# tennisonliu/bayesian-neural-network

Hardware: AMD Instinct MI355X
Metric: MC-forward-samples/sec + KL-elements/sec, 784-1200-1200-10 BNN (higher is better)
Workload: dtype bf16

## Files before the change

### bayesian-neural-network_amd/csrc/bbb_linear.hip

```cpp
#include "bnn_device.h"
#include "bnn_fin.h"
#include "bbb_sample_body.h"
#include "bbb_block_gemm.h"
#include "../../include/bnn_hip.h"
#include <string.h>

namespace bnn {

struct BbbK {
  const void* x;
  long x_sstride;
  const float* w_mu;
  const float* w_rho;
  const float* w_sigma;
  const float* b_mu;
  const float* b_rho;
  const float* eps_w;
  const float* eps_b;
  float* eps_w_dump;
  float* eps_b_dump;
  void* y;
  float4* ws;
  int S, B, K, N;
  __bf16* y16;
// ... 581 lines not shown
      if (threadIdx.x == 0) fp->ks_stats[(size_t)s * KS + ks] = make_float4(own0, own1, own2, 0.f);
      asm volatile("s_waitcnt vmcnt(0)" ::: "memory");
      __syncthreads();
      uint32_t* flag = reinterpret_cast<uint32_t*>(part);
      if (threadIdx.x == 0) {
        __builtin_amdgcn_fence(__ATOMIC_RELEASE, "agent");
        asm volatile("s_waitcnt vmcnt(0)" ::: "memory");
        const uint32_t tk = __hip_atomic_fetch_add(fp->ks_ticket + s, 1u, __ATOMIC_RELAXED, __HIP_MEMORY_SCOPE_AGENT);
        const uint32_t last = (tk == (uint32_t)KS - 1u) ? 1u : 0u;
        if (last) {
          __builtin_amdgcn_fence(__ATOMIC_ACQUIRE, "agent");
          asm volatile("s_waitcnt vmcnt(0)" ::: "memory");
        }
        *flag = last;
      }
      __syncthreads();
      BNN_STAMP(7);
      if (*flag == 0u) return true;
      __syncthreads();
      const float* tiles = fp->ks_tiles + (size_t)s * KS * (128 * 16);
      float4 q4 = make_float4(0.f, 0.f, 0.f, 0.f);
      if ((int)threadIdx.x < KS) q4 = fp->ks_stats[(size_t)s * KS + threadIdx.x];
      for (int it = threadIdx.x; it < 128 * 4; it += blockDim.x) {
        const int brow = it >> 2, fg = it & 3;
        f32x4 v = f32x4{0.f, 0.f, 0.f, 0.f};
        for (int j = 0; j < KS; ++j) v += *reinterpret_cast<const f32x4*>(tiles + (size_t)j * (128 * 16) + brow * 16 + fg * 4);
        if (p.relu) {
#pragma unroll
          for (int i = 0; i < 4; ++i) v[i] = fmaxf(v[i], 0.f);
        }
        *reinterpret_cast<f32x4*>(fin_lg + brow * 16 + fg * 4) = v;
        if (brow < B) {
          float* yp = reinterpret_cast<float*>(p.y) + ((size_t)s * B + brow) * N + fg * 4;
#pragma unroll
          for (int i = 0; i < 4; ++i)
            if (fg * 4 + i < N) yp[i] = v[i];
        }
      }
      if (threadIdx.x < 64) {
        own0 = wave_sum(q4.x);
        own1 = wave_sum(q4.y);
        own2 = wave_sum(q4.z);
      }
      if (threadIdx.x == 0) {
        p.ws[1 + (size_t)s * ntiles + nt] = make_float4(own0, own1, own2, 0.f);
        fp->ks_ticket[s] = 0u;
      }
    }
    __syncthreads();
    BNN_STAMP(10);
    float a = 0.f, b = 0.f, nll = 0.f;
    const int own_layer = fk.n_layers - 1;
#ifdef BNN_STAMPS
    fin_sample(fk, fp->c, s, T, fin_lg, 16, own_layer, own0, own1, own2, part, a, b, nll, p.dbg ? p.dbg + (size_t)blockIdx.x * 16 : nullptr);
#else
    fin_sample(fk, fp->c, s, T, fin_lg, 16, own_layer, own0, own1, own2, part, a, b, nll);
#endif
    BNN_STAMP(11);
    if (threadIdx.x == 0) {
      fin_store(fk, s, a, b, nll);
      if (fk.S == 1) {
        if (fp->sums) {
          float* so = fp->sums;
          so[0] = a; so[1] = b; so[2] = nll; so[3] = 1.f;
        }
        if (fk.sample_counter) *fk.sample_counter += fk.sample_counter_inc;
      } else if (fp->ticket) {
        fin_samples_meet(fk, fp->sums, fp->ticket);
      }
    }
  }
  return true;
}

template <int MATH, int XDT, int R, bool ALIGNED>
__global__ __launch_bounds__(768) void bbb_fwd_kernel(const BbbK p) {
  bbb_fwd_body<MATH, XDT, R, ALIGNED, false>(p, nullptr);
}

template <int MATH, int XDT, bool XTL = false>
__global__ __launch_bounds__(768) void bbb_fwd_final_kernel(const BbbK p, const FinPack fp) {
  bbb_fwd_body<MATH, XDT, 1, true, true, false, false, 8, false, XTL>(p, &fp);
}

template <int XDT, int R>
__global__ __launch_bounds__(768) void bbb_fwd_rider_kernel(const BbbK p, const SampleK sk, int n_main) {
  if ((int)blockIdx.x >= n_main) {
    extern __shared__ __attribute__((aligned(16))) float lds[];
    sample_block(sk, (int)blockIdx.x - n_main, lds);
    return;
  }
  bbb_fwd_body<BNN_MATH_BF16, XDT, R, true, false>(p, nullptr);
}

struct FinRows {
  const void* x;
  long x_sstride;
  int xg;
  const __bf16* w;
  const float* b;
  float* y;
  int S, B, K, N, relu;
  uint32_t* tickets;
  float* parts;
};

template <bool XF32>
__global__ __launch_bounds__(256) void bbb_final_rows_kernel(const FinRows p, const FinPack fp, const FinLoss tr) {
  __shared__ __attribute__((aligned(16))) f32x4 red[4][64];
  __shared__ float lg[16][17];
  __shared__ __attribute__((aligned(8))) float part[4 * kFinNV];
  const FinK& fk = fp.k;
  const int RB = (p.B + 15) >> 4;
  const int s = (int)blockIdx.x / (RB + 1), rb = (int)blockIdx.x - s * (RB + 1);
  const int lane = threadIdx.x & 63, wave = threadIdx.x >> 6;
  float pub0 = 0.f, pub1 = 0.f;
  int slot = rb;
  if (rb == RB) {
    int T[8];
#pragma unroll
    for (int l = 0; l < 8; ++l) T[l] = (l < fk.n_layers) ? __float_as_int(reinterpret_cast<const float4*>(fk.ws[l])[0].x) : 0;
    float a = 0.f, b = 0.f, nll = 0.f;
    fin_sample(fk, fp.c, s, T, nullptr, 0, -1, 0.f, 0.f, 0.f, part, a, b, nll);
    pub0 = a;
    pub1 = b;
    slot = 8;
  } else {
    const int r = lane & 15, q = lane >> 4;
    const int K = p.K, N = p.N, B = p.B;
    const int row = min(rb * 16 + r, B - 1);
    const size_t xoff = (size_t)(s / p.xg) * (size_t)p.x_sstride + (size_t)row * K;
    const __bf16* xr = reinterpret_cast<const __bf16*>(p.x) + xoff;
    const float* xr32 = reinterpret_cast<const float*>(p.x) + xoff;
    const __bf16* wr = p.w + ((size_t)s * N + min(r, N - 1)) * K;
    const int ksteps = (K + 31) >> 5;
    f32x4 acc = f32x4{0.f, 0.f, 0.f, 0.f};
    constexpr int U = 10;
    for (int base = wave; base < ksteps; base += 4 * U) {
      float4 xa[U], xh[XF32 ? U : 1], wa[U];
#pragma unroll
      for (int u = 0; u < U; ++u) {
        const int k = (base + 4 * u) * 32 + q * 8;
        const int kk = min(k, K - 8);
        if (XF32) {
          xa[u] = *reinterpret_cast<const float4*>(xr32 + kk);
          xh[u] = *reinterpret_cast<const float4*>(xr32 + kk + 4);
        } else {
          xa[u] = *reinterpret_cast<const float4*>(xr + kk);
        }
        wa[u] = *reinterpret_cast<const float4*>(wr + kk);
      }
#pragma unroll
      for (int u = 0; u < U; ++u) {
        const int k = (base + 4 * u) * 32 + q * 8;
        const bool ok = (base + 4 * u) < ksteps && k < K && r < N;
        const float4 wz = ok ? wa[u] : make_float4(0.f, 0.f, 0.f, 0.f);
        bf16x8 xb;
        if (XF32) {
          const float xv[8] = {xa[u].x, xa[u].y, xa[u].z, xa[u].w, xh[u].x, xh[u].y, xh[u].z, xh[u].w};
#pragma unroll
          for (int j = 0; j < 8; ++j) xb[j] = (__bf16)xv[j];
        } else {
          xb = __builtin_bit_cast(bf16x8, xa[u]);
        }
        acc = __builtin_amdgcn_mfma_f32_16x16x32_bf16(__builtin_bit_cast(bf16x8, wz), xb, acc, 0, 0, 0);
      }
// ... 1356 lines not shown
      }
    } else if (ride) {
      const unsigned n_main = grid.x;
      const dim3 grid_r(n_main + (unsigned)rider_blocks);
#define BNN_GEMM_EPS(KERNEL, SIGV, ...)                                                                        \
  do {                                                                                                         \
    if (k.eps_mode == BNN_EPS_PHILOX) hipLaunchKernelGGL((KERNEL<SIGV, BNN_EPS_PHILOX>), __VA_ARGS__);          \
    else if (k.eps_mode == BNN_EPS_MEMORY) hipLaunchKernelGGL((KERNEL<SIGV, BNN_EPS_MEMORY>), __VA_ARGS__);     \
    else hipLaunchKernelGGL((KERNEL<SIGV, BNN_EPS_ZERO>), __VA_ARGS__);                                         \
  } while (0)
      if (a->w_sigma) BNN_GEMM_EPS(bbb_fwd_gemm_rider_kernel, true, grid_r, block, 0, stream, k, sk, (int)n_main);
      else BNN_GEMM_EPS(bbb_fwd_gemm_rider_kernel, false, grid_r, block, 0, stream, k, sk, (int)n_main);
    } else if (a->w_sigma) {
      if (k.eps_mode == BNN_EPS_PHILOX) hipLaunchKernelGGL((bbb_fwd_gemm_kernel<4, true, BNN_EPS_PHILOX>), grid, block, 0, stream, k);
      else if (k.eps_mode == BNN_EPS_MEMORY) hipLaunchKernelGGL((bbb_fwd_gemm_kernel<4, true, BNN_EPS_MEMORY>), grid, block, 0, stream, k);
      else hipLaunchKernelGGL((bbb_fwd_gemm_kernel<4, true, BNN_EPS_ZERO>), grid, block, 0, stream, k);
    } else {
      if (k.eps_mode == BNN_EPS_PHILOX) hipLaunchKernelGGL((bbb_fwd_gemm_kernel<4, false, BNN_EPS_PHILOX>), grid, block, 0, stream, k);
      else if (k.eps_mode == BNN_EPS_MEMORY) hipLaunchKernelGGL((bbb_fwd_gemm_kernel<4, false, BNN_EPS_MEMORY>), grid, block, 0, stream, k);
      else hipLaunchKernelGGL((bbb_fwd_gemm_kernel<4, false, BNN_EPS_ZERO>), grid, block, 0, stream, k);
    }
#undef BNN_GEMM_EPS
  } else if (ride) {
    const unsigned n_main = (unsigned)(((pl.blocks + 7) / 8) * 8);
    const dim3 grid_r(n_main + (unsigned)rider_blocks);
    const size_t lds_r = pl.lds > kSampleRedFloats * sizeof(float) ? pl.lds : kSampleRedFloats * sizeof(float);
#define BNN_RIDE(XDT, RR)                                                                                    \
  do {                                                                                                       \
    err = allow_big_lds(bbb_fwd_rider_kernel<XDT, RR>, lds_r);                                               \
    if (err == hipSuccess)                                                                                   \
      hipLaunchKernelGGL((bbb_fwd_rider_kernel<XDT, RR>), grid_r, block, lds_r, stream, k, sk, (int)n_main); \
  } while (0)
#define BNN_RIDE_R(XDT)                          \
  do {                                           \
    if (pl.R == 1) BNN_RIDE(XDT, 1);             \
    else if (pl.R == 2) BNN_RIDE(XDT, 2);        \
    else BNN_RIDE(XDT, 4);                       \
  } while (0)
    if (xdt == BNN_F32) BNN_RIDE_R(BNN_F32); else BNN_RIDE_R(BNN_BF16);
#undef BNN_RIDE
#undef BNN_RIDE_R
    if (err != hipSuccess) return (int)err;
  } else {
#define BNN_GO(MATH, XDT, RR, AL)                                                              \
  do {                                                                                         \
    err = allow_big_lds(bbb_fwd_kernel<MATH, XDT, RR, AL>, pl.lds);                            \
    if (err == hipSuccess)                                                                     \
      hipLaunchKernelGGL((bbb_fwd_kernel<MATH, XDT, RR, AL>), grid, block, pl.lds, stream, k); \
  } while (0)
#define BNN_GO_R(MATH, XDT)                                   \
  do {                                                        \
    if (!al) BNN_GO(MATH, XDT, 1, false);                     \
    else if (pl.R == 1) BNN_GO(MATH, XDT, 1, true);           \
    else if (pl.R == 2) BNN_GO(MATH, XDT, 2, true);           \
    else BNN_GO(MATH, XDT, 4, true);                          \
  } while (0)
    if (math == BNN_MATH_BF16) {
      if (xdt == BNN_F32) BNN_GO_R(BNN_MATH_BF16, BNN_F32); else BNN_GO_R(BNN_MATH_BF16, BNN_BF16);
    } else if (math == BNN_MATH_BF16X3) {
      if (xdt == BNN_F32) BNN_GO_R(BNN_MATH_BF16X3, BNN_F32); else BNN_GO_R(BNN_MATH_BF16X3, BNN_BF16);
    } else {
      if (xdt == BNN_F32) BNN_GO_R(BNN_MATH_F32, BNN_F32); else BNN_GO_R(BNN_MATH_F32, BNN_BF16);
    }
#undef BNN_GO
#undef BNN_GO_R
    if (err != hipSuccess) return (int)err;
  }
  err = hipGetLastError();
  if (err != hipSuccess) return (int)err;
  if (a->log_prior || a->log_q) {
    hipLaunchKernelGGL(bbb_layer_scalars_kernel, dim3(a->n_samples), dim3(256), 0, stream, k.ws, K, a->out_features,
                       a->prior, a->log_prior, a->log_q);
    err = hipGetLastError();
    if (err != hipSuccess) return (int)err;
  }
  return BNN_OK;
}

extern "C" int bnn_bbb_linear_fwd(const bnn_bbb_fwd_args* a, void* stream_) {
  return bbb_linear_fwd_impl(a, stream_, false, nullptr, 0);
}

static constexpr int kFinalTicketMaxSamples = 16;
static constexpr int kRowsTicketMaxSamples = 64;

extern "C" size_t bnn_bbb_final_scratch_bytes(int32_t n_samples) {
  return n_samples <= 0 ? 0 : fin_scratch(nullptr, (size_t)n_samples).bytes;
}

extern "C" int bnn_bbb_final_fwd(const bnn_bbb_fwd_args* a, const bnn_finalize_args* f, void* stream_) {
  BbbK k;
  bool al = false;
  int rc = prepare(a, k, al);
  if (rc != BNN_OK) return rc;
  const bool x_pieces = a->x_layout == BNN_LAYOUT_PIECES;
  if (a->y_layout || a->w_pieces || (x_pieces && (a->w_sampled || a->math != BNN_MATH_BF16))) return BNN_ERR_ENUM;
  FinPack fp;
  rc = make_fin(f, fp.k, fp.c);
  if (rc != BNN_OK) return rc;
  const int nl = f->n_layers;
  rc = check_fin_loss(f);
  if (rc != BNN_OK) return rc;
  if (a->w_sampled) {
    const int S = a->n_samples, B = a->batch, N = a->out_features, K = a->in_features;
    const bool rows = a->y_dtype == BNN_F32 && N <= 16 && B <= 128 && S <= 4096 && !f->local_reparam &&
                      nl >= 1 && f->n_samples == S && f->classes == N && f->batch == B && f->logits == a->y && f->nll &&
                      f->scratch && f->scratch_bytes >= bnn_bbb_final_scratch_bytes(S) &&
                      !(reinterpret_cast<uintptr_t>(f->scratch) & 15) &&
                      (S == 1 || f->ticket || (S > kRowsTicketMaxSamples && !f->loss)) && !a->rider &&
                      (N % 4 != 0 || !(reinterpret_cast<uintptr_t>(a->y) & 15));
    if (!rows) {
      rc = bnn_bbb_linear_fwd(a, stream_);
      if (rc == BNN_OK) rc = bnn_elbo_finalize(f, stream_);
      return rc != BNN_OK ? rc : bnn_loss_tail_(f, stream_);
    }
    const FinLoss tr = make_fin_loss(f);
    FinRows fr;
    fr.x = a->x;
    fr.x_sstride = k.x_sstride; fr.xg = k.xg;
    fr.w = k.w_pre; fr.b = k.b_pre;
    fr.y = reinterpret_cast<float*>(a->y);
    fr.S = S; fr.B = B; fr.K = K; fr.N = N; fr.relu = a->relu ? 1 : 0;
    const FinScratch sc = fin_scratch(f->scratch, (size_t)S);
    fr.tickets = sc.tickets;
    fr.parts = sc.stats;
    const bool rows_tail = S > kRowsTicketMaxSamples && !tr.out4;
    fp.sums = f->sums;
    fp.ticket = rows_tail ? nullptr : f->ticket;
    fp.ks = 1; fp.ks_ticket = nullptr; fp.ks_stats = nullptr; fp.ks_tiles = nullptr;
    const int RB = (B + 15) / 16;
    if (a->x_dtype == BNN_BF16)
      hipLaunchKernelGGL(bbb_final_rows_kernel<false>, dim3((unsigned)(S * (RB + 1))), dim3(256), 0, reinterpret_cast<hipStream_t>(stream_),
                         fr, fp, tr);
    else
      hipLaunchKernelGGL(bbb_final_rows_kernel<true>, dim3((unsigned)(S * (RB + 1))), dim3(256), 0, reinterpret_cast<hipStream_t>(stream_),
                         fr, fp, tr);
    const hipError_t e2 = hipGetLastError();
    if (e2 != hipSuccess) return (int)e2;
    return rows_tail ? bnn_elbo_sums_(f, stream_) : (int)BNN_OK;
  }
  const bool fuse = al && a->out_features <= 16 && a->batch <= 128 && a->want_stats && !f->local_reparam && nl >= 1 &&
                    f->layer_workspace[nl - 1] == a->workspace && f->n_samples == a->n_samples &&
                    f->classes == a->out_features && f->batch == a->batch && a->y_dtype == BNN_F32 &&
                    (a->n_samples == 1 || a->n_samples > kFinalTicketMaxSamples || f->ticket != nullptr) && !(a->log_prior || a->log_q) &&
                    a->form == BNN_FORM_AUTO;
  if (x_pieces && !fuse) return BNN_ERR_ENUM;
  if (!fuse) {
    rc = bnn_bbb_linear_fwd(a, stream_);
    if (rc != BNN_OK) return rc;
    rc = bnn_elbo_finalize(f, stream_);
    return rc != BNN_OK ? rc : bnn_loss_tail_(f, stream_);
  }
  hipStream_t stream = reinterpret_cast<hipStream_t>(stream_);
  fp.sums = f->sums;
  const bool tail_kernel = a->n_samples > kFinalTicketMaxSamples;
  fp.ticket = tail_kernel ? nullptr : f->ticket;
  const int K = a->in_features;
  const int ssteps = (K + 31) / 32;
  if (x_pieces) k.x_sstride = a->x_per_sample ? (long)ssteps * 4096 : 0;
  int KS = (ssteps + 11) / 12;
  KS = KS > kFinalMaxSlices ? kFinalMaxSlices : KS;
  for (int ks = KS; ks <= kFinalMaxSlices; ++ks) {
    const int per = (ssteps + ks - 1) / ks;
    if (per <= 12 && ((per & 3) == 0 || per < 4)) {
      KS = ks;
      break;
    }
  }
  if ((long)a->n_samples * KS > 128) KS = 1;
  if (KS > 1 && (!f->scratch || f->scratch_bytes < bnn_bbb_final_scratch_bytes(a->n_samples) ||
                 (reinterpret_cast<uintptr_t>(f->scratch) & 15)))
    KS = 1;
  const int spb = (ssteps + KS - 1) / KS;
  int spw = 1;
  while ((spb + spw - 1) / spw > 12) ++spw;
  int nw = (spb + spw - 1) / spw;
  nw = nw < 1 ? 1 : nw;
  fp.ks = KS;
  const FinScratch sc = fin_scratch(f->scratch, (size_t)a->n_samples);
  fp.ks_ticket = sc.tickets;
  fp.ks_stats = reinterpret_cast<float4*>(sc.stats);
  fp.ks_tiles = sc.tiles;
  const long total = (long)a->n_samples * KS;
  hipError_t err = hipSuccess;
  const dim3 grid((unsigned)(((total + 7) / 8) * 8)), block(nw * 64);
  const size_t lds = ((size_t)nw * 8 * 64 * 4 + 16 + 3 * nw + 128 * 16 + kFinMaxWaves * kFinNV) * sizeof(float);
#define BNN_FIN(MATH, XDT)                                                                     \
  do {                                                                                         \
    err = allow_big_lds(bbb_fwd_final_kernel<MATH, XDT>, lds);                                 \
    if (err == hipSuccess)                                                                     \
      hipLaunchKernelGGL((bbb_fwd_final_kernel<MATH, XDT>), grid, block, lds, stream, k, fp);  \
  } while (0)
  if (x_pieces) {
    err = allow_big_lds(bbb_fwd_final_kernel<BNN_MATH_BF16, BNN_BF16, true>, lds);
    if (err == hipSuccess)
      hipLaunchKernelGGL((bbb_fwd_final_kernel<BNN_MATH_BF16, BNN_BF16, true>), grid, block, lds, stream, k, fp);
  } else if (a->math == BNN_MATH_BF16) {
    if (a->x_dtype == BNN_F32) BNN_FIN(BNN_MATH_BF16, BNN_F32); else BNN_FIN(BNN_MATH_BF16, BNN_BF16);
  } else if (a->math == BNN_MATH_BF16X3) {
    if (a->x_dtype == BNN_F32) BNN_FIN(BNN_MATH_BF16X3, BNN_F32); else BNN_FIN(BNN_MATH_BF16X3, BNN_BF16);
  } else {
    if (a->x_dtype == BNN_F32) BNN_FIN(BNN_MATH_F32, BNN_F32); else BNN_FIN(BNN_MATH_F32, BNN_BF16);
  }
#undef BNN_FIN
  if (err != hipSuccess) return (int)err;
  err = hipGetLastError();
  if (err != hipSuccess) return (int)err;
  rc = tail_kernel ? bnn_elbo_sums_(f, stream_) : (int)BNN_OK;
  return rc != BNN_OK ? rc : bnn_loss_tail_(f, stream_);
}

extern "C" int bnn_bbb_input_grad_(const bnn_bbb_bwd_args* a, const float* gz, void* stream_) {
  hipStream_t stream = reinterpret_cast<hipStream_t>(stream_);
  if (a->w_sampled_t) {
    if (a->math != BNN_MATH_BF16) return BNN_ERR_ENUM;
    bnn_bbb_fwd_args fa{};
    fa.struct_bytes = sizeof(bnn_bbb_fwd_args);
    fa.n_samples = a->n_samples; fa.batch = a->batch;
    fa.in_features = a->out_features;
    fa.out_features = a->in_features;
    const bool g16 = a->gy_bf16 && gz == a->gy;
    fa.x = g16 ? a->gy_bf16 : static_cast<const void*>(gz);
    fa.x_dtype = g16 ? BNN_BF16 : BNN_F32;
    fa.x_per_sample = 1;
    fa.math = BNN_MATH_BF16; fa.eps_mode = BNN_EPS_ZERO;
    fa.y = a->g_x; fa.y_dtype = BNN_F32;
    fa.y_bf16_copy = a->g_x_bf16;
    fa.w_sampled = a->w_sampled_t;
    fa.b_sampled = a->b_mu;
    fa.prior = a->prior;
    return bbb_linear_fwd_impl(&fa, stream_, true, a->gx_relu_mask ? a->x : nullptr,
                               a->x_per_sample ? (long)a->batch * a->in_features : 0);
  }
  BbbK k{};
  k.x = gz;
  k.x_sstride = (long)a->batch * a->out_features;
  k.w_mu = a->w_mu; k.w_rho = a->w_rho; k.b_mu = a->b_mu; k.b_rho = a->b_rho;
  k.w_sigma = nullptr;
  k.eps_w = a->eps_w; k.eps_b = a->eps_b; k.eps_w_dump = nullptr; k.eps_b_dump = nullptr;
  k.y = a->g_x;
  k.ws = nullptr;
  k.S = a->n_samples; k.B = a->batch;
  k.K = a->out_features;
  k.N = a->in_features;
  k.ldw = a->in_features;
  k.mask = a->gx_relu_mask ? a->x : nullptr;
  k.mask_sstride = a->x_per_sample ? (long)a->batch * a->in_features : 0;
  k.w_pre = reinterpret_cast<const __bf16*>(a->w_sampled);
  k.b_pre = nullptr;
  k.eps_mode = a->eps_mode; k.prior_kind = a->prior.kind; k.want_stats = 0; k.relu = 0; k.y_bf16 = 0; k.spb = 1;
  k.k0 = (uint32_t)a->seed; k.k1 = (uint32_t)(a->seed >> 32);
  k.layer_id = a->layer_id; k.sample_offset = a->sample_offset; k.sample_counter = a->sample_counter;
  k.xg = 1; k.sgrp = 0u; k.sgrp_stride = 0u;
  k.mix = PriorMix{};
#ifdef BNN_STAMPS
  k.dbg = nullptr;
#endif
  if ((a->in_features % 4 == 0) && (reinterpret_cast<uintptr_t>(a->g_x) & 15)) return BNN_ERR_ALIGN;
  const bool al = (k.K % 8 == 0) && aligned16(gz);
  BbbPlan pl{};
  tile_plan(k.S, k.B, k.K, k.N, al, 8, pl);
  const long total = pl.blocks;
  const dim3 grid((unsigned)(((total + 7) / 8) * 8)), block(pl.nw * 64);
  const size_t lds = pl.lds;
  hipError_t err = hipSuccess;
#define BNN_IG(MATH, RR, AL)                                                                    \
  do {                                                                                          \
    err = allow_big_lds(bbb_input_grad_kernel<MATH, RR, AL>, lds);                              \
    if (err == hipSuccess)                                                                      \
      hipLaunchKernelGGL((bbb_input_grad_kernel<MATH, RR, AL>), grid, block, lds, stream, k);   \
  } while (0)
#define BNN_IG_R(MATH)                                 \
  do {                                                 \
    if (!al) BNN_IG(MATH, 1, false);                   \
    else if (pl.R == 1) BNN_IG(MATH, 1, true);         \
    else if (pl.R == 2) BNN_IG(MATH, 2, true);         \
    else BNN_IG(MATH, 4, true);                        \
  } while (0)
#define BNN_IGP(RR, AL, MTT)                                                                         \
  do {                                                                                               \
    err = allow_big_lds(bbb_input_grad_pre_kernel<RR, AL, MTT>, ldsp);                               \
    if (err == hipSuccess)                                                                           \
      hipLaunchKernelGGL((bbb_input_grad_pre_kernel<RR, AL, MTT>), gridp, block, ldsp, stream, k);   \
  } while (0)
  if (a->w_sampled) {
    if (a->math != BNN_MATH_BF16) return BNN_ERR_ENUM;
    const long totalp = (long)((k.N + 15) / 16) * k.S * ((k.B + 127) / 128);
    const dim3 gridp((unsigned)(((totalp + 7) / 8) * 8));
    const size_t ldsp = pl.lds;
    if (!al) BNN_IGP(1, false, 8); else BNN_IGP(1, true, 8);
  } else if (a->math == BNN_MATH_BF16) BNN_IG_R(BNN_MATH_BF16); else BNN_IG_R(BNN_MATH_F32);
// ... 8 lines not shown
```

### bayesian-neural-network_amd/csrc/bnn_fin.h

```cpp
#pragma once
#include "bnn_device.h"
#include "bnn_prior.h"
#include "bnn_nll_row.h"
#include "../../include/bnn_hip.h"
#include <math.h>

extern "C" int bnn_elbo_sums_(const bnn_finalize_args* f, void* stream);
extern "C" int bnn_loss_tail_(const bnn_finalize_args* f, void* stream);

namespace bnn {

struct FinK {
  const float* ws[8];
  int lin[8], lout[8];
  int n_layers, local_reparam, S, B, C;
  bnn_prior prior;
  const float* logits;
  const void* target;
  int nll_mode;
  float nll_sigma;
  float *log_prior, *log_q, *kl, *nll;
  uint32_t* sample_counter;
  uint32_t sample_counter_inc;
  int group;
  long tgt_stride;
  const float* nll_partial;
  int nll_rb;
};

struct FinC {
  double cnt_c0[8];
  double lp_const[8];
  double kl_const[8];
  double inv2var;
  double reg_const;
  double reg_inv2var;
};

struct FinTail {
  FinK k;
  FinC c;
  float* sums;
  uint32_t* ticket;
};

constexpr int kFinNV = 25;
constexpr int kFinMaxWaves = 16;
constexpr int kFinalMaxSlices = 8;

struct FinScratch {
  uint32_t* tickets;
  float* stats;
  float* tiles;
  size_t bytes;
};
static inline FinScratch fin_scratch(void* base, size_t S) {
  const size_t tickets = ((S * 4 + 255) / 256) * 256, stats = S * kFinalMaxSlices * 16, tiles = S * kFinalMaxSlices * (128 * 16 * 4);
  const uintptr_t b = reinterpret_cast<uintptr_t>(base);
  return {reinterpret_cast<uint32_t*>(b), reinterpret_cast<float*>(b + tickets), reinterpret_cast<float*>(b + tickets + stats),
          tickets + stats + tiles};
}

static inline int make_fin(const bnn_finalize_args* a, FinK& k, FinC& cst) {
  if (!a) return BNN_ERR_NULL;
  if (a->struct_bytes != sizeof(bnn_finalize_args)) return BNN_ERR_ABI;
  if (a->n_layers < 0 || a->n_layers > 8 || a->n_samples <= 0 || a->n_samples > 65535) return BNN_ERR_SHAPE;
  if (prior_check(a->prior) == BNN_ERR_ENUM || (unsigned)a->nll_mode > 1u) return BNN_ERR_ENUM;
  for (int l = 0; l < 8; ++l) {
    k.ws[l] = l < a->n_layers ? reinterpret_cast<const float*>(a->layer_workspace[l]) : nullptr;
    k.lin[l] = l < a->n_layers ? a->layer_in[l] : 0;
    k.lout[l] = l < a->n_layers ? a->layer_out[l] : 0;
    if (l < a->n_layers) {
      if (!k.ws[l]) return BNN_ERR_NULL;
      if (reinterpret_cast<uintptr_t>(k.ws[l]) & 15) return BNN_ERR_ALIGN;
      if (k.lin[l] <= 0 || k.lout[l] <= 0) return BNN_ERR_SHAPE;
    }
  }
  if (a->n_layers > 0 && a->prior.kind != BNN_PRIOR_MIXTURE && prior_check(a->prior) != BNN_OK) return BNN_ERR_SHAPE;
  if (a->group_samples < 0 || (a->group_samples > 0 && a->n_samples % a->group_samples != 0)) return BNN_ERR_SHAPE;
  if (a->target_per_group && a->group_samples <= 0) return BNN_ERR_SHAPE;
  if (a->nll) {
    if (!a->logits || !a->target) return BNN_ERR_NULL;
    if (a->batch <= 0 || a->classes <= 0) return BNN_ERR_SHAPE;
    if (a->nll_mode == BNN_NLL_REGRESSION && !(a->nll_sigma > 0.f)) return BNN_ERR_SHAPE;
  }
  k.n_layers = a->n_layers; k.local_reparam = a->local_reparam; k.S = a->n_samples; k.B = a->batch; k.C = a->classes;
  k.prior = a->prior; k.logits = a->logits; k.target = a->target; k.nll_mode = a->nll_mode;
  k.nll_sigma = a->nll_sigma; k.log_prior = a->log_prior; k.log_q = a->log_q; k.kl = a->kl; k.nll = a->nll;
  k.sample_counter = a->sample_counter; k.sample_counter_inc = a->sample_counter_inc;
  k.group = a->group_samples;
  k.nll_partial = nullptr; k.nll_rb = 0;
  k.tgt_stride = a->target_per_group
                     ? (a->nll_mode == BNN_NLL_CLASSIFICATION ? (long)a->batch : (long)a->batch * a->classes) : 0;
  for (int l = 0; l < 8; ++l) cst.cnt_c0[l] = cst.lp_const[l] = cst.kl_const[l] = 0.0;
  for (int l = 0; l < a->n_layers; ++l) {
    const PriorFold f = prior_fold_make(a->prior, (double)a->layer_out[l] * a->layer_in[l] + a->layer_out[l]);
    cst.cnt_c0[l] = f.cnt_c0;
    cst.lp_const[l] = f.lp_const;
    cst.kl_const[l] = f.kl_const;
  }
  cst.inv2var = prior_fold_make(a->prior, 0.0).inv2var;
  const double ns = a->nll_sigma > 0.f ? (double)a->nll_sigma : 1.0;
  cst.reg_const = log(ns) - kNegLogSqrt2Pi;
  cst.reg_inv2var = 1.0 / (2.0 * ns * ns);
  return BNN_OK;
}

__device__ __forceinline__ float fin_nll(const FinK& p, const FinC& cst, int s, const float* lg, int ldc, int row0, int row1) {
  const int lane = threadIdx.x & 63, wave = threadIdx.x >> 6;
  float acc = 0.f;
    if (p.nll_mode == BNN_NLL_CLASSIFICATION) {
    const long long* tgt = reinterpret_cast<const long long*>(p.target) + (p.group > 0 ? (s / p.group) * p.tgt_stride : 0);
    if (p.C <= 32) {
      for (int b = row0 + (int)threadIdx.x; b < row1; b += blockDim.x) {
        const float* row = lg + (size_t)b * ldc;
        const long long tc = tgt[b];
        float mx, se = 0.f;
        if (ldc == 16 && p.C <= 16) {
          float vr[16];
#pragma unroll
          for (int i = 0; i < 16; ++i) vr[i] = row[(i + b) & 15];
          mx = -3.0e38f;
#pragma unroll
          for (int i = 0; i < 16; ++i) mx = (((i + b) & 15) < p.C) ? fmaxf(mx, vr[i]) : mx;
#pragma unroll
          for (int i = 0; i < 16; ++i) se += (((i + b) & 15) < p.C) ? __expf(vr[i] - mx) : 0.f;
          se = __logf(se);
        } else if (p.C <= 16) {
          float vr[16];
#pragma unroll
          for (int i = 0; i < 16; ++i) vr[i] = row[min(i, p.C - 1)];
          mx = vr[0];
#pragma unroll
          for (int i = 1; i < 16; ++i) mx = i < p.C ? fmaxf(mx, vr[i]) : mx;
#pragma unroll
          for (int i = 0; i < 16; ++i) se += i < p.C ? __expf(vr[i] - mx) : 0.f;
          se = __logf(se);
        } else {
          mx = row[0];
          for (int cc = 1; cc < p.C; ++cc) mx = fmaxf(mx, row[cc]);
          for (int cc = 0; cc < p.C; ++cc) se += expf(row[cc] - mx);
          se = logf(se);
        }
        const float picked = (tc >= 0 && tc < p.C) ? row[tc] : __builtin_nanf("");
        acc += (mx + se) - picked;
      }
    } else {
      const int nwv = blockDim.x >> 6;
      for (int b = row0 + wave; b < row1; b += nwv) {
        const float* row = lg + (size_t)b * ldc;
        float mx = -3.0e38f;
#pragma unroll 8
        for (int cc = lane; cc < p.C; cc += 64) mx = fmaxf(mx, row[cc]);
#pragma unroll
        for (int off = 32; off > 0; off >>= 1) mx = fmaxf(mx, __shfl_xor(mx, off, 64));
        float se = 0.f;
#pragma unroll 8
        for (int cc = lane; cc < p.C; cc += 64) se += __expf(row[cc] - mx);
        se = wave_sum(se);
        if (lane == 0) {
          const long long tc = tgt[b];
          const float picked = (tc >= 0 && tc < p.C) ? row[tc] : __builtin_nanf("");
          acc += (mx + logf(se)) - picked;
        }
      }
    }
  } else {
    const float* tgt = reinterpret_cast<const float*>(p.target) + (p.group > 0 ? (s / p.group) * p.tgt_stride : 0);
    if (p.C <= 8) {
      for (int b = row0 + (int)threadIdx.x; b < row1; b += blockDim.x)
        for (int cc = 0; cc < p.C; ++cc) {
          const float d = tgt[(size_t)b * p.C + cc] - lg[(size_t)b * ldc + cc];
          acc += (float)((double)(d * d) * cst.reg_inv2var + cst.reg_const);
        }
    } else {
      const int nwv = blockDim.x >> 6;
      float d2 = 0.f;
      int cnt = 0;
      for (int b = row0 + wave; b < row1; b += nwv) {
        const float* row = lg + (size_t)b * ldc;
        const float* trow = tgt + (size_t)b * p.C;
        if (((p.C | ldc) & 3) == 0 && ((reinterpret_cast<uintptr_t>(row) | reinterpret_cast<uintptr_t>(trow)) & 15) == 0) {
#pragma unroll 4
          for (int cc = lane * 4; cc < p.C; cc += 256) {
            const float4 t4 = *reinterpret_cast<const float4*>(trow + cc), r4 = *reinterpret_cast<const float4*>(row + cc);
            const float dx = t4.x - r4.x, dy = t4.y - r4.y, dz = t4.z - r4.z, dw = t4.w - r4.w;
            d2 = __builtin_fmaf(dx, dx, __builtin_fmaf(dy, dy, __builtin_fmaf(dz, dz, __builtin_fmaf(dw, dw, d2))));
            cnt += 4;
          }
        } else {
#pragma unroll 8
          for (int cc = lane; cc < p.C; cc += 64) {
            const float d = trow[cc] - row[cc];
            d2 = __builtin_fmaf(d, d, d2);
            ++cnt;
          }
        }
      }
      acc = (float)((double)d2 * cst.reg_inv2var + (double)cnt * cst.reg_const);
    }
  }
  return acc;
}

__device__ __forceinline__ float fin_row_nll(const FinK& fk, const FinC& cst, int s, int brow, const float* lgrow) {
  const int C = fk.C;
  float acc_n = 0.f;
  if (fk.nll_mode == BNN_NLL_CLASSIFICATION) {
    const long long* tgt = reinterpret_cast<const long long*>(fk.target) + (fk.group > 0 ? (s / fk.group) * fk.tgt_stride : 0);
    const long long tc = tgt[brow];
    float mx = -3.0e38f, se = 0.f;
    for (int c = 0; c < C; ++c) mx = fmaxf(mx, lgrow[c]);
    for (int c = 0; c < C; ++c) se += __expf(lgrow[c] - mx);
    const float picked = (tc >= 0 && tc < C) ? lgrow[(int)tc] : __builtin_nanf("");
    acc_n = (mx + __logf(se)) - picked;
  } else {
    const float* tgt = reinterpret_cast<const float*>(fk.target) + (fk.group > 0 ? (s / fk.group) * fk.tgt_stride : 0);
    for (int c = 0; c < C; ++c) {
      const float d = tgt[(size_t)brow * C + c] - lgrow[c];
      acc_n += (float)((double)(d * d) * cst.reg_inv2var + cst.reg_const);
    }
  }
  return acc_n;
}

__device__ __forceinline__ void fin_sample(const FinK& p, const FinC& cst, int s, const int T[8], const float* lg, int ldc,
                                           int own_layer, float own0, float own1, float own2, float* part,
                                           float& out_a, float& out_b, float& out_nll, unsigned long long* dbg = nullptr) {
#define FIN_STAMP(i) do { if (dbg && threadIdx.x == 0) dbg[i] = __builtin_amdgcn_s_memtime(); } while (0)
  constexpr int NV = kFinNV;
  const int lane = threadIdx.x & 63, wave = threadIdx.x >> 6;
  float v[NV];
#pragma unroll
  for (int i = 0; i < NV; ++i) v[i] = 0.f;
#pragma unroll
  for (int l = 0; l < 8; ++l) {
    if (l < p.n_layers && l != own_layer) {
      const float4* ws = reinterpret_cast<const float4*>(p.ws[l]);
      const int Tl = T[l], bd = blockDim.x;
      constexpr int FU = 8;
      for (int t0 = threadIdx.x; t0 < Tl; t0 += FU * bd) {
        float4 qv[FU];
        float lsz[FU];
#pragma unroll
        for (int u = 0; u < FU; ++u) {
          const int t = min(t0 + u * bd, Tl - 1);
          qv[u] = p.local_reparam ? ws[1 + t] : ws[1 + (size_t)s * Tl + t];
          lsz[u] = p.local_reparam ? 0.f : ws[1 + t].z;
        }
#pragma unroll
        for (int u = 0; u < FU; ++u) {
          if (t0 + u * bd < Tl) {
            v[3 * l + 0] += qv[u].x;
            v[3 * l + 1] += qv[u].y;
            v[3 * l + 2] += p.local_reparam ? qv[u].z : lsz[u];
          }
        }
      }
    }
  }
  FIN_STAMP(12);
  if (p.nll && p.nll_partial) {
    float acc = 0.f;
    for (int t = threadIdx.x; t < p.nll_rb; t += blockDim.x) acc += p.nll_partial[(size_t)s * p.nll_rb + t];
    v[NV - 1] = acc;
  } else if (p.nll && lg) {
    v[NV - 1] = fin_nll(p, cst, s, lg, ldc, 0, p.B);
  }
  FIN_STAMP(13);
  const int nv = 3 * p.n_layers;
  if (nv <= 9) {
    float t[10];
#pragma unroll
    for (int i = 0; i < 9; ++i) t[i] = wave_sum(v[i]);
    t[9] = wave_sum(v[NV - 1]);
    if (lane == 0) {
#pragma unroll
      for (int i = 0; i < 9; ++i) part[wave * NV + i] = t[i];
      part[wave * NV + NV - 1] = t[9];
    }
  } else {
#pragma unroll
    for (int i = 0; i < NV; ++i) {
      if (i < nv || i == NV - 1) {
        const float t = wave_sum(v[i]);
        if (lane == 0) part[wave * NV + i] = t;
      }
    }
  }
  FIN_STAMP(14);
  __syncthreads();
  double folded = 0;
  {
    const int nwv = blockDim.x >> 6;
    if ((int)threadIdx.x < NV && ((int)threadIdx.x < nv || (int)threadIdx.x == NV - 1))
      for (int w = 0; w < nwv; ++w) folded += (double)part[w * NV + threadIdx.x];
  }
  __syncthreads();
  if ((int)threadIdx.x < NV) reinterpret_cast<double*>(part)[threadIdx.x] = folded;
  __syncthreads();
  FIN_STAMP(15);
  if (threadIdx.x == 0) {
    auto red = [&](int i) { return reinterpret_cast<const double*>(part)[i]; };
    float a_tot = 0.f, b_tot = 0.f;
#pragma unroll
    for (int l = 0; l < 8; ++l) {
      if (l >= p.n_layers) break;
      double r0, r1, r2;
      if (l == own_layer) {
        r0 = own0; r1 = own1; r2 = own2;
      } else {
        r0 = red(3 * l); r1 = red(3 * l + 1); r2 = red(3 * l + 2);
      }
      if (p.local_reparam) {
        a_tot += (float)(cst.kl_const[l] - r0 + (r1 + r2) * cst.inv2var);
      } else {
        const double lq = fold_log_q(cst.cnt_c0[l], r2, r0);
        const double lp = fold_log_p(p.prior.kind, cst.lp_const[l], cst.inv2var, r1);
        a_tot += (float)lp;
        b_tot += (float)lq;
      }
    }
    out_a = a_tot;
    out_b = b_tot;
    out_nll = (float)red(NV - 1);
  }
}

template <typename Emit>
__device__ __forceinline__ void fin_fold_groups(const float* pa, const float* pb, const float* pn, int S, int g, Emit emit) {
  const float* fb = pa ? pa : pb ? pb : pn;
  double ta = 0, tb = 0, tn = 0;
  int left = g, group = 0;
  constexpr int CH = 16;
  for (int base = 0; base < S; base += CH) {
    float va[CH], vb[CH], vn[CH];
    if (fb) {
      const float* qa = pa ? pa : fb;
      const float* qb = pb ? pb : fb;
      const float* qn = pn ? pn : fb;
#pragma unroll
      for (int j = 0; j < CH; ++j) {
        const int i = min(base + j, S - 1);
        va[j] = __hip_atomic_load(qa + i, __ATOMIC_RELAXED, __HIP_MEMORY_SCOPE_AGENT);
        vb[j] = __hip_atomic_load(qb + i, __ATOMIC_RELAXED, __HIP_MEMORY_SCOPE_AGENT);
        vn[j] = __hip_atomic_load(qn + i, __ATOMIC_RELAXED, __HIP_MEMORY_SCOPE_AGENT);
      }
    } else {
#pragma unroll
      for (int j = 0; j < CH; ++j) va[j] = vb[j] = vn[j] = 0.f;
    }
#pragma unroll
    for (int j = 0; j < CH; ++j) {
      if (base + j < S) {
        ta += pa ? va[j] : 0.f;
        tb += pb ? vb[j] : 0.f;
        tn += pn ? vn[j] : 0.f;
        if (--left == 0) {
          emit(group, ta, tb, tn);
          ta = tb = tn = 0;
          left = g;
          ++group;
        }
      }
    }
  }
}

__device__ __forceinline__ void fin_fold_sums(const FinK& p, float* sums) {
  const int g = p.group > 0 ? p.group : p.S;
  const float* pa = p.local_reparam ? p.kl : p.log_prior;
  const float* pb = (!p.local_reparam && p.log_q) ? p.log_q : nullptr;
  fin_fold_groups(pa, pb, p.nll, p.S, g, [&](int m, double ta, double tb, double tn) {
    float* so = sums + 4 * m;
    so[0] = (float)ta; so[1] = (float)tb; so[2] = (float)tn; so[3] = (float)g;
  });
}

__device__ __forceinline__ void fin_store(const FinK& p, int s, float a, float b, float nll) {
  if (p.local_reparam) {
    if (p.kl) p.kl[s] = a;
  } else {
    if (p.log_prior) p.log_prior[s] = a;
    if (p.log_q) p.log_q[s] = b;
  }
  if (p.nll) p.nll[s] = nll;
}

struct FinLoss {
  const float* beta;
  float total, grad_scale, inv_var;
  float* out4;
  float* g_a;
  float* g_b;
  float* g_kl3;
  float* g_logits;
};

__device__ __forceinline__ void fin_loss_assemble(const FinK& fk, const FinLoss& tr) {
  const float* pa = fk.local_reparam ? fk.kl : fk.log_prior;
  double x = 0, y = 0, z = 0;
  fin_fold_groups(pa, fk.local_reparam ? nullptr : fk.log_q, fk.nll, fk.S, fk.S, [&](int, double ta, double tb, double tn) { x = ta; y = tb; z = tn; });
  const float beta = *tr.beta;
  const float inv = tr.grad_scale / tr.total;
  for (int i = 0; i < fk.S; ++i) {
    if (tr.g_a) tr.g_a[i] = fk.local_reparam ? 0.f : -beta * inv;
    if (tr.g_b) tr.g_b[i] = beta * inv;
  }
  const float am = (float)x / tr.total, bm = (float)y / tr.total, nm = (float)z / tr.total;
// ... 89 lines not shown
```

Baseline: 533,900.

## Add specialized final-layer kernel with prefetched finalize inputs and fused ELBO sums

Adds a dedicated final-layer forward kernel for the piece-layout, Gaussian-prior, single-split case. It prefetches weight parameters and activations one step ahead, and issues the finalize-stage loads (per-layer KL partials and target rows) before the GEMM loop so their latency overlaps compute. When samples are ungrouped, it also writes the per-sample ELBO sums and handles the ticket in-kernel, which skips the separate elbo_sums launch. In exchange there is more specialized code and higher register pressure, and the ticket-completion path is duplicated.

After: 535,700 (median of 6 runs). About the same (+0.3%).

```diff
diff --git a/bayesian-neural-network_amd/csrc/bbb_linear.hip b/bayesian-neural-network_amd/csrc/bbb_linear.hip
--- a/bayesian-neural-network_amd/csrc/bbb_linear.hip
+++ b/bayesian-neural-network_amd/csrc/bbb_linear.hip
@@ -687,6 +687,10 @@
 __global__ __launch_bounds__(768) void bbb_fwd_final_kernel(const BbbK p, const FinPack fp) {
   bbb_fwd_body<MATH, XDT, 1, true, true, false, false, 8, false, XTL>(p, &fp);
 }
+
+}
+#include "bbb_pair_final.h"
+namespace bnn {
 
 template <int XDT, int R>
 __global__ __launch_bounds__(768) void bbb_fwd_rider_kernel(const BbbK p, const SampleK sk, int n_main) {
@@ -2209,6 +2213,9 @@
 }
 
 static constexpr int kFinalTicketMaxSamples = 16;
+#ifndef BNN_PAIR_FINAL_PARTS
+#define BNN_PAIR_FINAL_PARTS 3
+#endif
 static constexpr int kRowsTicketMaxSamples = 64;
 
 extern "C" size_t bnn_bbb_final_scratch_bytes(int32_t n_samples) {
@@ -2309,6 +2316,10 @@
   fp.ks_stats = reinterpret_cast<float4*>(sc.stats);
   fp.ks_tiles = sc.tiles;
   const long total = (long)a->n_samples * KS;
+  const bool pair_kernel = (BNN_PAIR_FINAL_PARTS & 1) && x_pieces && tail_kernel && KS == 1 && a->prior.kind == BNN_PRIOR_GAUSS &&
+                           !k.eps_w_dump && !k.eps_b_dump && !k.wt_out && !f->loss;
+  const bool pair_sums = (BNN_PAIR_FINAL_PARTS & 2) && pair_kernel && f->group_samples == 1 && f->sums && f->ticket;
+  if (pair_sums) fp.ticket = f->ticket;
   hipError_t err = hipSuccess;
   const dim3 grid((unsigned)(((total + 7) / 8) * 8)), block(nw * 64);
   const size_t lds = ((size_t)nw * 8 * 64 * 4 + 16 + 3 * nw + 128 * 16 + kFinMaxWaves * kFinNV) * sizeof(float);
@@ -2318,7 +2329,15 @@
     if (err == hipSuccess)                                                                     \
       hipLaunchKernelGGL((bbb_fwd_final_kernel<MATH, XDT>), grid, block, lds, stream, k, fp);  \
   } while (0)
-  if (x_pieces) {
+  if (pair_kernel) {
+    if (a->eps_mode == BNN_EPS_PHILOX) {
+      err = allow_big_lds(bbb_pair_final_kernel<true>, lds);
+      if (err == hipSuccess) hipLaunchKernelGGL(bbb_pair_final_kernel<true>, grid, block, lds, stream, k, fp);
+    } else {
+      err = allow_big_lds(bbb_pair_final_kernel<false>, lds);
+      if (err == hipSuccess) hipLaunchKernelGGL(bbb_pair_final_kernel<false>, grid, block, lds, stream, k, fp);
+    }
+  } else if (x_pieces) {
     err = allow_big_lds(bbb_fwd_final_kernel<BNN_MATH_BF16, BNN_BF16, true>, lds);
     if (err == hipSuccess)
       hipLaunchKernelGGL((bbb_fwd_final_kernel<BNN_MATH_BF16, BNN_BF16, true>), grid, block, lds, stream, k, fp);
@@ -2333,7 +2352,7 @@
   if (err != hipSuccess) return (int)err;
   err = hipGetLastError();
   if (err != hipSuccess) return (int)err;
-  rc = tail_kernel ? bnn_elbo_sums_(f, stream_) : (int)BNN_OK;
+  rc = (tail_kernel && !pair_sums) ? bnn_elbo_sums_(f, stream_) : (int)BNN_OK;
   return rc != BNN_OK ? rc : bnn_loss_tail_(f, stream_);
 }
 
diff --git a/bayesian-neural-network_amd/csrc/bbb_pair_final.h b/bayesian-neural-network_amd/csrc/bbb_pair_final.h
--- /dev/null
+++ b/bayesian-neural-network_amd/csrc/bbb_pair_final.h
@@ -0,0 +1,187 @@
+#pragma once
+
+namespace bnn {
+
+template <bool PHILOX>
+__global__ __launch_bounds__(768) void bbb_pair_final_kernel(const BbbK p, const FinPack fp) {
+  extern __shared__ __attribute__((aligned(16))) float lds[];
+  const int lane = threadIdx.x & 63, wave = threadIdx.x >> 6, nw = blockDim.x >> 6;
+  const int n = lane & 15, q = lane >> 4;
+  const int K = p.K, N = p.N, B = p.B;
+  int s;
+  if (!xcd_work_item(p.S, s)) return;
+  const bool n_ok = n < N;
+  const int nc = min(n, N - 1);
+  const int mtiles = min(8, (B + 15) >> 4);
+  const int ssteps = (K + 31) / 32;
+  const FinK& fk = fp.k;
+  const int own_layer = fk.n_layers - 1;
+  const char* xs = reinterpret_cast<const char*>(p.x) + (size_t)(s / p.xg) * (size_t)p.x_sstride * 2;
+
+  float* lds_bias = lds + (size_t)nw * 8 * 64 * 4;
+  float* lds_red = lds_bias + 16;
+  f32x4* slab = reinterpret_cast<f32x4*>(lds);
+
+  BNN_STAMP(0);
+  BNN_STAMP_RT(8);
+  auto load_x = [&](int t, float4 (&xr)[8]) {
+#pragma unroll
+    for (int m = 0; m < 8; ++m) xr[m] = *reinterpret_cast<const float4*>(xs + ((size_t)((t * 8 + m) * 64 + lane)) * 16);
+  };
+  auto load_params = [&](int t, float (&mu)[8], float (&rho)[8]) {
+    const size_t woff = (size_t)nc * K + min(t * 32 + q * 8, K - 8);
+    load8<true>(p.w_mu + woff, 8, mu);
+    load8<true>(p.w_rho + woff, 8, rho);
+  };
+  float4 xr[8];
+  float mu_n[8], rho_n[8];
+  if (wave < ssteps) {
+    load_params(wave, mu_n, rho_n);
+    load_x(wave, xr);
+  }
+  int T[8];
+#pragma unroll
+  for (int l = 0; l < 8; ++l) {
+    const int tl = __float_as_int(reinterpret_cast<const float4*>(fk.ws[l < own_layer ? l : own_layer])[0].x);
+    T[l] = l < own_layer ? tl : 0;
+  }
+  const uint32_t gs = global_sample(p, s);
+  const int gpr = (int)eps_groups_per_row(K);
+  const uint32_t wid = eps_tensor_id(p.layer_id, kEpsWeight);
+
+  float bmu_pre = 0.f, brho_pre = 0.f, beps_pre = 0.f;
+  if (wave == nw - 1 && lane < 16 && n_ok) {
+    bmu_pre = p.b_mu[n];
+    brho_pre = p.b_rho[n];
+    if constexpr (PHILOX) beps_pre = eps_bias(n, gs, p.layer_id, p.k0, p.k1);
+    else beps_pre = bias_eps(p, n, s, gs, false);
+  }
+
+  FinPre pre;
+  fin_request(fk, s, T, own_layer, true, nw * 64, pre);
+
+  f32x4 acc[8];
+#pragma unroll
+  for (int m = 0; m < 8; ++m) acc[m] = f32x4{0.f, 0.f, 0.f, 0.f};
+  float s_e2 = 0.f, s_a = 0.f, s_ls = 0.f;
+  uint32_t tk = 0u;
+
+#pragma nounroll
+  for (int t = wave; t < ssteps; t += nw) {
+    const int k = t * 32 + q * 8;
+    const int valid = n_ok ? min(8, K - k) : 0;
+    float mu[8], sg[8];
+#pragma unroll
+    for (int j = 0; j < 8; ++j) {
+      mu[j] = mu_n[j];
+      sg[j] = rho_n[j];
+    }
+    if (t + nw < ssteps) load_params(t + nw, mu_n, rho_n);
+    if (t == wave) { asm volatile("" :: "v"(mu[0]), "v"(sg[0])); BNN_STAMP(1); }
+
+    float e[8], w[8];
+    if constexpr (PHILOX) {
+      const uint32_t g = eps_group((uint32_t)n, k, (uint32_t)gpr);
+      philox_normal8(g, gs, wid, p.k0, p.k1, e);
+    } else if (p.eps_mode == BNN_EPS_MEMORY) {
+      load8<true>(p.eps_w + ((size_t)s * N + n) * K + k, valid, e);
+    } else {
+#pragma unroll
+      for (int j = 0; j < 8; ++j) e[j] = 0.f;
+    }
+    float e2 = 0.f, a = 0.f, ls = 0.f;
+#pragma unroll
+    for (int j = 0; j < 8; ++j) {
+      sg[j] = softplus(sg[j]);
+      w[j] = __builtin_fmaf(sg[j], e[j], mu[j]);
+      e2 = __builtin_fmaf(e[j], e[j], e2);
+    }
+#pragma unroll
+    for (int j = 0; j < 8; ++j) a = __builtin_fmaf(w[j], w[j], a);
+#pragma unroll
+    for (int j = 0; j < 8; ++j) ls = add_log(ls, sg[j]);
+    const bool lane_ok = valid > 0;
+    s_e2 += lane_ok ? e2 : 0.f;
+    s_a += lane_ok ? a : 0.f;
+    s_ls += lane_ok ? ls : 0.f;
+    if (valid <= 0) {
+#pragma unroll
+      for (int j = 0; j < 8; ++j) w[j] = 0.f;
+    }
+    if (t == wave) { asm volatile("" :: "v"(w[0]), "v"(w[7])); BNN_STAMP(2); }
+    if (t == wave && threadIdx.x == 0 && fp.ticket) {
+      uint32_t one = 1u;
+      asm volatile("" : "+v"(one) : "v"(e[0]));
+      tk = __hip_atomic_fetch_add(fp.ticket, one, __ATOMIC_RELAXED, __HIP_MEMORY_SCOPE_AGENT);
+    }
+    bf16x8 wa;
+#pragma unroll
+    for (int j = 0; j < 8; ++j) wa[j] = (__bf16)w[j];
+#pragma unroll
+    for (int m = 0; m < 8; ++m)
+      acc[m] = __builtin_amdgcn_mfma_f32_16x16x32_bf16(wa, __builtin_bit_cast(bf16x8, xr[m]), acc[m], 0, 0, 0);
+    if (t + nw < ssteps) load_x(t + nw, xr);
+  }
+
+  asm volatile("" :: "v"(acc[0][0]), "v"(acc[7][3]));
+  BNN_STAMP(3);
+  if (wave == nw - 1 && lane < 16) {
+    float b = 0.f;
+    if (n_ok) b = sample_bias(p, bmu_pre, brho_pre, beps_pre, true, true, s_e2, s_a, s_ls);
+    lds_bias[lane] = b;
+  }
+#pragma unroll
+  for (int m = 0; m < 8; ++m)
+    if (m < mtiles) slab[(wave * 8 + m) * 64 + lane] = acc[m];
+  {
+    const float a = wave_sum(s_e2), b = wave_sum(s_a), cc = wave_sum(s_ls);
+    if (lane == 0) {
+      lds_red[wave * 3 + 0] = a;
+      lds_red[wave * 3 + 1] = b;
+      lds_red[wave * 3 + 2] = cc;
+    }
+  }
+  BNN_STAMP(4);
+  __syncthreads();
+  BNN_STAMP(5);
+  float own0 = 0.f, own1 = 0.f, own2 = 0.f;
+  if (threadIdx.x == 0) {
+    for (int wv = 0; wv < nw; ++wv) {
+      own0 += lds_red[wv * 3 + 0];
+      own1 += lds_red[wv * 3 + 1];
+      own2 += lds_red[wv * 3 + 2];
+    }
+    if (s == 0) p.ws[0] = make_float4(__int_as_float(1), 0.f, 0.f, 0.f);
+    p.ws[1 + (size_t)s] = make_float4(own0, own1, own2, 0.f);
+  }
+  float* fin_lg = lds_red + 3 * nw;
+  epilogue_store<1, 8>(p, slab, lds_bias, nw, mtiles, 0, s, 0, fin_lg);
+  BNN_STAMP(6);
+  BNN_STAMP_RT(9);
+  float* part = reinterpret_cast<float*>((reinterpret_cast<uintptr_t>(fin_lg + 128 * 16) + 7) & ~(uintptr_t)7);
+  __syncthreads();
+  BNN_STAMP(10);
+  float a = 0.f, b = 0.f, nll = 0.f;
+#ifdef BNN_STAMPS
+  fin_fold(fk, fp.c, s, T, pre, fin_lg, 16, own_layer, own0, own1, own2, part, a, b, nll, p.dbg ? p.dbg + (size_t)blockIdx.x * 16 : nullptr);
+#else
+  fin_fold(fk, fp.c, s, T, pre, fin_lg, 16, own_layer, own0, own1, own2, part, a, b, nll);
+#endif
+  BNN_STAMP(11);
+  if (threadIdx.x == 0) {
+    fin_store(fk, s, a, b, nll);
+    if (fp.ticket) {
+      float* so = fp.sums + 4 * (size_t)s;
+      so[0] = fk.log_prior ? a : 0.f;
+      so[1] = fk.log_q ? b : 0.f;
+      so[2] = fk.nll ? nll : 0.f;
+      so[3] = 1.f;
+      if (tk == (uint32_t)fk.S - 1u) {
+        __hip_atomic_store(fp.ticket, 0u, __ATOMIC_RELAXED, __HIP_MEMORY_SCOPE_AGENT);
+        if (fk.sample_counter) *fk.sample_counter += fk.sample_counter_inc;
+      }
+    }
+  }
+}
+
+}
diff --git a/bayesian-neural-network_amd/csrc/bnn_fin.h b/bayesian-neural-network_amd/csrc/bnn_fin.h
--- a/bayesian-neural-network_amd/csrc/bnn_fin.h
+++ b/bayesian-neural-network_amd/csrc/bnn_fin.h
@@ -106,15 +106,26 @@
   return BNN_OK;
 }
 
-__device__ __forceinline__ float fin_nll(const FinK& p, const FinC& cst, int s, const float* lg, int ldc, int row0, int row1) {
+constexpr int kFinPreLayers = 2;
+struct FinPre {
+  float4 q[kFinPreLayers];
+  float lsz[kFinPreLayers];
+  bool have[kFinPreLayers];
+  bool have_row;
+  long long row;
+};
+
+__device__ __forceinline__ float fin_nll(const FinK& p, const FinC& cst, int s, const float* lg, int ldc, int row0, int row1,
+                                         const FinPre* pre = nullptr) {
   const int lane = threadIdx.x & 63, wave = threadIdx.x >> 6;
+  const bool pre_row = pre && pre->have_row;
   float acc = 0.f;
     if (p.nll_mode == BNN_NLL_CLASSIFICATION) {
     const long long* tgt = reinterpret_cast<const long long*>(p.target) + (p.group > 0 ? (s / p.group) * p.tgt_stride : 0);
     if (p.C <= 32) {
       for (int b = row0 + (int)threadIdx.x; b < row1; b += blockDim.x) {
         const float* row = lg + (size_t)b * ldc;
-        const long long tc = tgt[b];
+        const long long tc = (pre_row && b == (int)threadIdx.x) ? pre->row : tgt[b];
         float mx, se = 0.f;
         if (ldc == 16 && p.C <= 16) {
           float vr[16];
@@ -170,7 +181,8 @@
     if (p.C <= 8) {
       for (int b = row0 + (int)threadIdx.x; b < row1; b += blockDim.x)
         for (int cc = 0; cc < p.C; ++cc) {
-          const float d = tgt[(size_t)b * p.C + cc] - lg[(size_t)b * ldc + cc];
+          const float tg = (pre_row && b == (int)threadIdx.x) ? __uint_as_float((uint32_t)pre->row) : tgt[(size_t)b * p.C + cc];
+          const float d = tg - lg[(size_t)b * ldc + cc];
           acc += (float)((double)(d * d) * cst.reg_inv2var + cst.reg_const);
         }
     } else {
@@ -224,18 +236,59 @@
   return acc_n;
 }
 
-__device__ __forceinline__ void fin_sample(const FinK& p, const FinC& cst, int s, const int T[8], const float* lg, int ldc,
-                                           int own_layer, float own0, float own1, float own2, float* part,
-                                           float& out_a, float& out_b, float& out_nll, unsigned long long* dbg = nullptr) {
+__device__ __forceinline__ void fin_request(const FinK& p, int s, const int T[8], int own_layer, bool rows, int bd, FinPre& pre) {
+#pragma unroll
+  for (int l = 0; l < kFinPreLayers; ++l) {
+    pre.q[l] = make_float4(0.f, 0.f, 0.f, 0.f);
+    pre.lsz[l] = 0.f;
+    pre.have[l] = l < p.n_layers && l != own_layer && T[l] > 0 && T[l] <= bd;
+    if (pre.have[l]) {
+      const float4* ws = reinterpret_cast<const float4*>(p.ws[l]);
+      const int Tl = T[l], t = min((int)threadIdx.x, Tl - 1);
+      pre.q[l] = p.local_reparam ? ws[1 + t] : ws[1 + (size_t)s * Tl + t];
+      pre.lsz[l] = p.local_reparam ? 0.f : ws[1 + t].z;
+    }
+  }
+  pre.have_row = false;
+  pre.row = 0;
+  if (rows && p.nll && !p.nll_partial && (int)threadIdx.x < p.B) {
+    const long g = p.group > 0 ? (s / p.group) * p.tgt_stride : 0;
+    if (p.nll_mode == BNN_NLL_CLASSIFICATION && p.C <= 32) {
+      pre.row = (reinterpret_cast<const long long*>(p.target) + g)[threadIdx.x];
+      pre.have_row = true;
+    } else if (p.nll_mode == BNN_NLL_REGRESSION && p.C == 1) {
+      pre.row = (long long)__float_as_uint((reinterpret_cast<const float*>(p.target) + g)[threadIdx.x]);
+      pre.have_row = true;
+    }
+  }
+}
+
+__device__ __forceinline__ void fin_fold(const FinK& p, const FinC& cst, int s, const int T[8], const FinPre& pre, const float* lg,
+                                         int ldc, int own_layer, float own0, float own1, float own2, float* part,
+                                         float& out_a, float& out_b, float& out_nll, unsigned long long* dbg = nullptr) {
 #define FIN_STAMP(i) do { if (dbg && threadIdx.x == 0) dbg[i] = __builtin_amdgcn_s_memtime(); } while (0)
   constexpr int NV = kFinNV;
   const int lane = threadIdx.x & 63, wave = threadIdx.x >> 6;
   float v[NV];
 #pragma unroll
   for (int i = 0; i < NV; ++i) v[i] = 0.f;
+  bool walk[8];
+#pragma unroll
+  for (int l = 0; l < 8; ++l) walk[l] = l < p.n_layers && l != own_layer;
+#pragma unroll
+  for (int l = 0; l < kFinPreLayers; ++l) {
+    if (pre.have[l]) {
+      walk[l] = false;
+      if ((int)threadIdx.x < T[l]) {
+        v[3 * l + 0] += pre.q[l].x;
+        v[3 * l + 1] += pre.q[l].y;
+        v[3 * l + 2] += p.local_reparam ? pre.q[l].z : pre.lsz[l];
+      }
+    }
+  }
 #pragma unroll
   for (int l = 0; l < 8; ++l) {
-    if (l < p.n_layers && l != own_layer) {
+    if (walk[l]) {
       const float4* ws = reinterpret_cast<const float4*>(p.ws[l]);
       const int Tl = T[l], bd = blockDim.x;
       constexpr int FU = 8;
@@ -265,7 +318,7 @@
     for (int t = threadIdx.x; t < p.nll_rb; t += blockDim.x) acc += p.nll_partial[(size_t)s * p.nll_rb + t];
     v[NV - 1] = acc;
   } else if (p.nll && lg) {
-    v[NV - 1] = fin_nll(p, cst, s, lg, ldc, 0, p.B);
+    v[NV - 1] = fin_nll(p, cst, s, lg, ldc, 0, p.B, &pre);
   }
   FIN_STAMP(13);
   const int nv = 3 * p.n_layers;
@@ -325,6 +378,14 @@
     out_b = b_tot;
     out_nll = (float)red(NV - 1);
   }
+}
+
+__device__ __forceinline__ void fin_sample(const FinK& p, const FinC& cst, int s, const int T[8], const float* lg, int ldc,
+                                           int own_layer, float own0, float own1, float own2, float* part,
+                                           float& out_a, float& out_b, float& out_nll, unsigned long long* dbg = nullptr) {
+  FinPre pre;
+  fin_request(p, s, T, own_layer, lg != nullptr, (int)blockDim.x, pre);
+  fin_fold(p, cst, s, T, pre, lg, ldc, own_layer, own0, own1, own2, part, out_a, out_b, out_nll, dbg);
 }
 
 template <typename Emit>
```
